# stevewongv/Sparse2Dense

Hardware: AMD Instinct MI355X
Metric: LiDAR frames/sec (fwd+bwd), 150k-pt 0.1m-voxel synthetic Waymo scene (higher is better)
Workload: dtype bf16 (sparse stack: bf16 storage; dense neck/head: bf16 NHWC activations; fp32 accumulate, statistics, master weights, optimizer)

## Files before the change

include/s2d.h:

```cpp
#ifndef S2D_H_
#define S2D_H_

#include <stddef.h>
#include <stdint.h>

#ifdef __cplusplus
extern "C" {
#endif

typedef void *s2d_stream_t;

#define S2D_OK 0
#define S2D_ERR_INVALID_ARG (-1)
#define S2D_ERR_UNSUPPORTED (-2)
#define S2D_ERR_CAPACITY (-3)
#define S2D_ERR_WORKSPACE (-4)
#define S2D_ERR_COMM (-5)

int s2d_version(void);
int s2d_last_error(char *buf, size_t buf_len);
int s2d_build_info(char *buf, size_t buf_len);

size_t s2d_voxelize_batch_workspace_bytes(int frames, const int64_t *point_offsets, int max_points, int max_voxels);
int s2d_voxelize_batch_run(const float *points, int frames, const int64_t *point_offsets, int ndim,
// ... 511 lines not shown
int s2d_comm_ranks(void);
int s2d_comm_shutdown(void);
int s2d_comm_allreduce_sum_f32(float *buf, int64_t count, s2d_stream_t stream);

int s2d_conv2d_pack_batch_bf16(int n, const float *const *weights, const int32_t *cin, const int32_t *cout, const int32_t *taps,
                               const int32_t *weight_nhwc, const int32_t *transpose_flip, void *const *packed_fwd, void *const *packed_dgrad,
                               s2d_stream_t stream);

int s2d_convt3d_mfma_fwd_stats_y16(const float *in, const void *packed, const float *bias, int batch, int cin, int cout, int d, int h, int w,
                                   void *out_bf16, float *stats_partial, s2d_stream_t stream);
int s2d_pointwise_conv_wgrad_norm_x16(const void *in_bf16, const float *in_scale_shift, const float *dout, int batch, int cin, int cout,
                                      int64_t positions, float *dweight, float *dbias, void *ws, size_t ws_bytes, s2d_stream_t stream);
int s2d_pcr_level_site_cache(void *buf, size_t bytes);
int s2d_pcr_level_fwd_y16_z16(const void *y, const float *bn_scale_shift, const float *head_params, const float *w2, const float *b2,
                              const int32_t *coors, const float *feats, int64_t m, int batch, int c, int co, int d, int h, int w, void *z_bf16,
                              float *z_stats, float *out8, void *ws, size_t ws_bytes, s2d_stream_t stream);
int s2d_pcr_level_bwd_sums_y16_z16(const void *y, const float *bn_scale_shift, const float *head_params, const int32_t *coors, const float *feats,
                                   int64_t m, int batch, int c, int d, int h, int w, const float *fwd_out8, const float *go_mask,
                                   const float *go_offset, const void *dz_bf16, const float *w2, int co, float *grads, float *bn_sums, void *ws,
                                   size_t ws_bytes, s2d_stream_t stream);
int s2d_pcr_level_bwd_apply_y16_d16_z16(const void *y, const float *bn_scale_shift, const float *head_params, const int32_t *coors,
                                        const float *feats, int64_t m, int batch, int c, int d, int h, int w, const float *fwd_out8,
                                        const float *go_mask, const float *go_offset, const void *dz_bf16, const float *w2, int co,
                                        const float *abd, void *dy_bf16, s2d_stream_t stream);
int s2d_pointwise_conv_wgrad_norm_x16_d16(const void *in_bf16, const float *in_scale_shift, const void *dout_bf16, int batch, int cin, int cout,
                                          int64_t positions, float *dweight, float *dbias, void *ws, size_t ws_bytes, s2d_stream_t stream);
int s2d_convt3d_mfma_x16_supported(int cin, int cout, int d, int h, int w);
int s2d_convt3d_mfma_fwd_stats_y16_norm_x16(const void *in_bf16, const float *in_scale_shift, const void *packed, const float *bias, int batch,
                                            int cin, int cout, int d, int h, int w, void *out_bf16, float *stats_partial, s2d_stream_t stream);
int s2d_convt3d_mfma_wgrad_d16_norm_x16(const void *in_bf16, const float *in_scale_shift, const void *dout_bf16, int batch, int cin, int cout,
                                        int d, int h, int w, float *dweight, void *ws, size_t ws_bytes, s2d_stream_t stream);
int s2d_convt3d_mfma_dgrad_d16_x16(const void *dout_bf16, const void *packed, int batch, int cin, int cout, int d, int h, int w, void *din_bf16,
                                   s2d_stream_t stream);
int s2d_bncm_bwd_reduce_x_typed(const void *dy, int dy_bf16, const void *x, int x_bf16, const float *scale, const float *shift, int batch, int c,
                                int64_t positions, float *sums, void *ws, size_t ws_bytes, s2d_stream_t stream);
int s2d_bncm_bwd_apply_x_typed(const void *dy, int dy_bf16, const void *x, int x_bf16, const float *scale, const float *shift, const float *a,
                               const float *b, const float *d, int batch, int c, int64_t positions, void *dx, int dx_bf16, s2d_stream_t stream);
int s2d_pcr_level_fwd_y16(const void *y, const float *bn_scale_shift, const float *head_params, const float *w2, const float *b2,
                          const int32_t *coors, const float *feats, int64_t m, int batch, int c, int co, int d, int h, int w, float *z,
                          float *z_stats, float *out8, void *ws, size_t ws_bytes, s2d_stream_t stream);
int s2d_pcr_level_bwd_sums_y16(const void *y, const float *bn_scale_shift, const float *head_params, const int32_t *coors, const float *feats,
                               int64_t m, int batch, int c, int d, int h, int w, const float *fwd_out8, const float *go_mask,
                               const float *go_offset, const float *dz, const float *w2, int co, float *grads, float *bn_sums, void *ws,
                               size_t ws_bytes, s2d_stream_t stream);
int s2d_pcr_level_bwd_apply_y16(const void *y, const float *bn_scale_shift, const float *head_params, const int32_t *coors, const float *feats,
                                int64_t m, int batch, int c, int d, int h, int w, const float *fwd_out8, const float *go_mask,
                                const float *go_offset, const float *dz, const float *w2, int co, const float *abd, float *dy,
                                s2d_stream_t stream);
int s2d_pcr_level_bwd_apply_y16_d16(const void *y, const float *bn_scale_shift, const float *head_params, const int32_t *coors, const float *feats,
                                    int64_t m, int batch, int c, int d, int h, int w, const float *fwd_out8, const float *go_mask,
                                    const float *go_offset, const float *dz, const float *w2, int co, const float *abd, void *dy_bf16,
                                    s2d_stream_t stream);

int s2d_pfn_supported(int ndim, int slots, int feats, int cout);
int s2d_pfn_blocks(int64_t pillars);
int s2d_pfn_bwd_cols(void);
int s2d_pfn_stats_f32(const float *voxels, const int32_t *num_points, const int32_t *coors, const float *weight, int64_t pillars,
                      int slots, int ndim, float vx, float vy, float x_offset, float y_offset, float *partial, s2d_stream_t stream);
int s2d_pfn_apply_max_f32(const float *voxels, const int32_t *num_points, const int32_t *coors, const float *weight, const float *scale,
                          const float *shift, int64_t pillars, int slots, int ndim, float vx, float vy, float x_offset, float y_offset,
                          float *out, uint8_t *argmax, s2d_stream_t stream);
int s2d_pfn_bwd_f32(const float *voxels, const int32_t *num_points, const int32_t *coors, const float *weight, const float *dout,
                    const uint8_t *argmax, int64_t pillars, int slots, int ndim, float vx, float vy, float x_offset, float y_offset,
                    float *partial, s2d_stream_t stream);

int s2d_pfn2_supported(int ndim, int slots, int feats, int c1, int c2);
// ... 177 lines not shown
```

sparse2dense_amd/_lib.py:

```python
import ctypes
import os

_HERE = os.path.dirname(os.path.abspath(__file__))
LIB_PATH = os.path.join(_HERE, "lib", "libs2d_hip.so")

c_i32p = ctypes.c_void_p
c_f32p = ctypes.c_void_p
_I3 = ctypes.c_int32 * 3
_PFN_GEO = [ctypes.c_int64, ctypes.c_int, ctypes.c_int, ctypes.c_float, ctypes.c_float, ctypes.c_float, ctypes.c_float]
_F3 = ctypes.c_float * 3
_F6 = ctypes.c_float * 6


class CenterTask(ctypes.Structure):
    _fields_ = [(n, ctypes.c_void_p) for n in ("hm_logit", "reg", "height", "dim", "vel", "rot", "hm", "ind", "mask", "cat", "anno_box", "p",
                                               "d_logit", "d_reg", "d_height", "d_dim", "d_vel", "d_rot")] + [("classes", ctypes.c_int)]

class CenterPredictTask(ctypes.Structure):
    _fields_ = [("map", ctypes.c_void_p * 6), ("channel_stride", ctypes.c_int64 * 6), ("pixel_stride", ctypes.c_int64 * 6),
                ("classes", ctypes.c_int), ("label_base", ctypes.c_int)]


class AnchorPredictTask(ctypes.Structure):
    _fields_ = [(n, ctypes.c_void_p) for n in ("box_preds", "cls_preds", "dir_cls_preds", "anchors")] + \
# ... 347 lines not shown
                                                 ctypes.c_int, ctypes.c_int, ctypes.c_int, ctypes.c_void_p, c_f32p, ctypes.c_void_p]),
    "s2d_conv2d3x3_wgrad_supported": (ctypes.c_int, [ctypes.c_int, ctypes.c_int]),
    "s2d_conv2d3x3_wgrad_workspace_bytes": (ctypes.c_size_t, [ctypes.c_int] * 6),
    "s2d_conv2d3x3_wgrad_nhwc_bf16": (ctypes.c_int, [ctypes.c_void_p, ctypes.c_void_p, ctypes.c_void_p] + [ctypes.c_int] * 6 +
                                      [c_f32p, c_f32p, ctypes.c_void_p, ctypes.c_size_t, ctypes.c_void_p]),
    "s2d_convt3d_k4s2p1_fwd_f32": (ctypes.c_int, [c_f32p, c_f32p, c_f32p, ctypes.c_int, ctypes.c_int, ctypes.c_int,
                                                  ctypes.c_int, ctypes.c_int, ctypes.c_int, c_f32p, ctypes.c_void_p]),
    "s2d_convt3d_k4s2p1_dgrad_f32": (ctypes.c_int, [c_f32p, c_f32p, ctypes.c_int, ctypes.c_int, ctypes.c_int,
                                                    ctypes.c_int, ctypes.c_int, ctypes.c_int, c_f32p, ctypes.c_void_p]),
    "s2d_convt3d_k4s2p1_wgrad_workspace_bytes": (ctypes.c_size_t, [ctypes.c_int] * 6),
    "s2d_convt3d_k4s2p1_wgrad_f32": (ctypes.c_int, [c_f32p, c_f32p, ctypes.c_int, ctypes.c_int, ctypes.c_int, ctypes.c_int,
                                                    ctypes.c_int, ctypes.c_int, c_f32p, ctypes.c_void_p, ctypes.c_size_t,
                                                    ctypes.c_void_p]),
    "s2d_bncm_workspace_bytes": (ctypes.c_size_t, [ctypes.c_int, ctypes.c_int, ctypes.c_int64]),
    "s2d_bncm_stats_f32": (ctypes.c_int, [c_f32p, ctypes.c_int, ctypes.c_int, ctypes.c_int64, c_f32p, ctypes.c_void_p,
                                          ctypes.c_size_t, ctypes.c_void_p]),
    "s2d_bncm_apply_f32": (ctypes.c_int, [c_f32p, c_f32p, c_f32p, ctypes.c_int, ctypes.c_int, ctypes.c_int,
                                          ctypes.c_int64, c_f32p, ctypes.c_void_p]),
    "s2d_bncm_bwd_reduce_f32": (ctypes.c_int, [c_f32p, c_f32p, c_f32p, ctypes.c_int, ctypes.c_int, ctypes.c_int,
                                               ctypes.c_int64, c_f32p, ctypes.c_void_p, ctypes.c_size_t, ctypes.c_void_p]),
    "s2d_bncm_bwd_reduce_x_f32": (ctypes.c_int, [c_f32p, c_f32p, c_f32p, c_f32p, ctypes.c_int, ctypes.c_int, ctypes.c_int64, c_f32p, ctypes.c_void_p,
                                                 ctypes.c_size_t, ctypes.c_void_p]),
    "s2d_bncm_bwd_apply_x_f32": (ctypes.c_int, [c_f32p] * 7 + [ctypes.c_int, ctypes.c_int, ctypes.c_int64, c_f32p, ctypes.c_void_p]),
    "s2d_bncm_bwd_reduce_x_typed": (ctypes.c_int, [ctypes.c_void_p, ctypes.c_int, ctypes.c_void_p, ctypes.c_int, c_f32p, c_f32p, ctypes.c_int, ctypes.c_int,
                                                   ctypes.c_int64, c_f32p, ctypes.c_void_p, ctypes.c_size_t, ctypes.c_void_p]),
    "s2d_bncm_bwd_apply_x_typed": (ctypes.c_int, [ctypes.c_void_p, ctypes.c_int, ctypes.c_void_p, ctypes.c_int, c_f32p, c_f32p, c_f32p, c_f32p, c_f32p,
                                                  ctypes.c_int, ctypes.c_int, ctypes.c_int64, ctypes.c_void_p, ctypes.c_int, ctypes.c_void_p]),
    "s2d_convt3d_mfma_x16_supported": (ctypes.c_int, [ctypes.c_int] * 5),
    "s2d_convt3d_mfma_dgrad_d16_x16": (ctypes.c_int, [ctypes.c_void_p, ctypes.c_void_p] + [ctypes.c_int] * 6 + [ctypes.c_void_p, ctypes.c_void_p]),
    "s2d_convt3d_mfma_fwd_stats_y16_norm_x16": (ctypes.c_int, [ctypes.c_void_p, c_f32p, ctypes.c_void_p, c_f32p] + [ctypes.c_int] * 6 +
                                                [ctypes.c_void_p, c_f32p, ctypes.c_void_p]),
    "s2d_convt3d_mfma_wgrad_d16_norm_x16": (ctypes.c_int, [ctypes.c_void_p, c_f32p, ctypes.c_void_p] + [ctypes.c_int] * 6 +
                                            [c_f32p, ctypes.c_void_p, ctypes.c_size_t, ctypes.c_void_p]),
    "s2d_pcr_level_site_cache": (ctypes.c_int, [ctypes.c_void_p, ctypes.c_size_t]),
    "s2d_pcr_level_fwd_y16_z16": (ctypes.c_int, [c_f32p, c_f32p, c_f32p, c_f32p, c_f32p, c_i32p, c_f32p, ctypes.c_int64] + [ctypes.c_int] * 6 +
                                  [ctypes.c_void_p, c_f32p, c_f32p, ctypes.c_void_p, ctypes.c_size_t, ctypes.c_void_p]),
    "s2d_pcr_level_bwd_sums_y16_z16": (ctypes.c_int, [c_f32p, c_f32p, c_f32p, c_i32p, c_f32p, ctypes.c_int64] + [ctypes.c_int] * 5 +
                                       [c_f32p, c_f32p, c_f32p, ctypes.c_void_p, c_f32p, ctypes.c_int, c_f32p, c_f32p, ctypes.c_void_p, ctypes.c_size_t,
                                        ctypes.c_void_p]),
    "s2d_pcr_level_bwd_apply_y16_d16_z16": (ctypes.c_int, [c_f32p, c_f32p, c_f32p, c_i32p, c_f32p, ctypes.c_int64] + [ctypes.c_int] * 5 +
                                            [c_f32p, c_f32p, c_f32p, ctypes.c_void_p, c_f32p, ctypes.c_int, c_f32p, ctypes.c_void_p, ctypes.c_void_p]),
    "s2d_pointwise_conv_wgrad_norm_x16_d16": (ctypes.c_int, [ctypes.c_void_p, c_f32p, ctypes.c_void_p, ctypes.c_int, ctypes.c_int, ctypes.c_int,
                                                              ctypes.c_int64, c_f32p, c_f32p, ctypes.c_void_p, ctypes.c_size_t, ctypes.c_void_p]),
    "s2d_space_depth2_nhwc_bf16": (ctypes.c_int, [ctypes.c_void_p] + [ctypes.c_int] * 5 + [ctypes.c_void_p, ctypes.c_void_p]),
    "s2d_bncm_bwd_apply_f32": (ctypes.c_int, [c_f32p, c_f32p, c_f32p, c_f32p, c_f32p, c_f32p, ctypes.c_int, ctypes.c_int,
                                              ctypes.c_int, ctypes.c_int64, c_f32p, ctypes.c_void_p]),
    "s2d_densify_bev_fwd_bf16": (ctypes.c_int, [ctypes.c_void_p, ctypes.c_int, c_i32p, ctypes.c_int64, ctypes.c_int, _I3,
                                                ctypes.c_int, ctypes.c_void_p, ctypes.c_void_p]),
    "s2d_densify_bev_bwd_bf16": (ctypes.c_int, [ctypes.c_void_p, c_i32p, ctypes.c_int64, ctypes.c_int, _I3, ctypes.c_int,
                                                ctypes.c_void_p, ctypes.c_int, ctypes.c_void_p]),
    "s2d_spconv_s16_wgrad": (ctypes.c_int, [ctypes.c_void_p, ctypes.c_int64, ctypes.c_void_p, c_i32p, ctypes.c_int64, ctypes.c_int,
                                            ctypes.c_int, ctypes.c_int, c_f32p, ctypes.c_void_p, ctypes.c_size_t, ctypes.c_void_p]),
    "s2d_densify_fwd_f32": (ctypes.c_int, [c_f32p, c_i32p, ctypes.c_int64, ctypes.c_int, _I3, ctypes.c_int, c_f32p,
                                           ctypes.c_void_p]),
    "s2d_densify_bwd_f32": (ctypes.c_int, [c_f32p, c_i32p, ctypes.c_int64, ctypes.c_int, _I3, ctypes.c_int, c_f32p,
                                           ctypes.c_void_p]),
    "s2d_anchor_assign_workspace_bytes": (ctypes.c_size_t, [ctypes.c_int, ctypes.c_int]),
    "s2d_anchor_assign": (ctypes.c_int, [c_f32p, c_i32p, ctypes.c_int, ctypes.c_int, c_f32p, ctypes.c_int64, ctypes.c_int, ctypes.c_int,
                                         ctypes.POINTER(ctypes.c_float), ctypes.POINTER(ctypes.c_float), c_i32p, c_f32p, c_f32p, ctypes.c_void_p,
                                         ctypes.c_size_t, ctypes.c_void_p]),
    "s2d_anchor_loss_workspace_bytes": (ctypes.c_size_t, [ctypes.c_int]),
    "s2d_anchor_loss_fwd": (ctypes.c_int, [c_f32p, c_f32p, c_f32p, c_i32p, c_f32p, c_f32p, ctypes.c_int, ctypes.c_int64, ctypes.c_int,
                                           ctypes.POINTER(ctypes.c_float), c_f32p, c_f32p, ctypes.c_void_p, ctypes.c_size_t, ctypes.c_void_p]),
    "s2d_anchor_loss_bwd": (ctypes.c_int, [c_f32p, c_f32p, c_f32p, c_i32p, c_f32p, c_f32p, ctypes.c_int, ctypes.c_int64, ctypes.c_int,
                                           ctypes.POINTER(ctypes.c_float), c_f32p, c_f32p, c_f32p, c_f32p, c_f32p, ctypes.c_void_p]),
    "s2d_anchor_decode": (ctypes.c_int, [c_f32p, c_f32p, c_f32p, c_f32p, ctypes.c_int, ctypes.c_int64, ctypes.c_int, ctypes.c_float, c_f32p,
# ... 158 lines not shown
```

sparse2dense_amd/csrc/convt3d_mfma.hip:

```cpp
#include "s2d_common.h"
#include <algorithm>
#include <cstdlib>

namespace s2d {

typedef float f32x4m __attribute__((ext_vector_type(4)));
typedef __bf16 bf16x8m __attribute__((ext_vector_type(8)));

constexpr unsigned CT_OOB = BUF_OOB;
__device__ __forceinline__ __amdgpu_buffer_rsrc_t ct_rsrc(const void *base, unsigned bytes) { return buf_rsrc(base, bytes); }
__device__ __forceinline__ f32x4m ct_load4(__amdgpu_buffer_rsrc_t r, unsigned voff, unsigned soff) { return buf_load4(r, voff, soff); }
typedef uint32_t u32x2m __attribute__((ext_vector_type(2)));
typedef uint32_t u32x3m __attribute__((ext_vector_type(3)));
typedef uint32_t u32x4m __attribute__((ext_vector_type(4)));
__device__ __forceinline__ u32x3m ct_load3u(__amdgpu_buffer_rsrc_t r, unsigned voff, unsigned soff) {
    return __builtin_bit_cast(u32x3m, __builtin_amdgcn_raw_buffer_load_b96(r, voff, soff, 0));
}
__device__ __forceinline__ u32x4m ct_load4u(__amdgpu_buffer_rsrc_t r, unsigned voff, unsigned soff) {
    return __builtin_bit_cast(u32x4m, __builtin_amdgcn_raw_buffer_load_b128(r, voff, soff, 0));
}
__device__ __forceinline__ u32x2m ct_load2u(__amdgpu_buffer_rsrc_t r, unsigned voff, unsigned soff) {
    return __builtin_bit_cast(u32x2m, __builtin_amdgcn_raw_buffer_load_b64(r, voff, soff, 0));
}
__device__ __forceinline__ uint32_t ct_hi_hi(uint32_t a, uint32_t b) { return __builtin_amdgcn_perm(b, a, 0x07060302u); }
// ... 1312 lines not shown
        const int a = f % CIT, g = f / CIT;
        const int ci = a * 16 + 4 * (ln >> 4) + reg, n_col = ln & 15;
        const int oc = n_col >> 2, okx = n_col & 3;
        if (ci < s.cin && oc < s.cout) dst[(((int64_t)ci * s.cout + oc) * 16 + g) * 4 + okx] = red[f4][ln];
    }
}

__global__ __launch_bounds__(256) void ct_slab_reduce_kernel(const float *__restrict__ partial, int n_slabs, int64_t size, float *__restrict__ out) {
    __shared__ float red[16][17];
    const int o = threadIdx.x & 15, sl = threadIdx.x >> 4;
    const int64_t i = (int64_t)blockIdx.x * 16 + o;
    float sum = 0.f;
    if (i < size)
        for (int sidx = sl; sidx < n_slabs; sidx += 16) sum += partial[(int64_t)sidx * size + i];
    red[sl][o] = sum;
    __syncthreads();
    if (sl == 0 && i < size) {
        float tot = 0.f;
#pragma unroll
        for (int k = 0; k < 16; ++k) tot += red[k][o];
        out[i] = tot;
    }
}

static bool ct_mfma_ok(int cin, int cout) { return (cin == 32 || cin == 16) && cout >= 1 && cout <= 32; }
static int ct_wgrad_blocks(int64_t rows) { return (int)(rows < 512 ? rows : 512); }
static bool ct_wgrad_is_narrow(int cout, int w) { return cout <= 4 && w % 8 == 0; }
static int ct_wgrad_blocks_for(int64_t rows, int cout, int w) {
    if (ct_wgrad_is_narrow(cout, w)) return (int)(rows < 1024 ? rows : 1024);
    if (w % 4 == 0) return (int)(rows < 128 ? rows : 128);
    return ct_wgrad_blocks(rows);
}

}

using namespace s2d;

extern "C" int s2d_convt3d_mfma_supported(int cin, int cout) { return ct_mfma_ok(cin, cout); }

extern "C" size_t s2d_convt3d_mfma_packed_elems(int cin, int cout) {
    if (!ct_mfma_ok(cin, cout)) return 0;
    const int nt_f = (cout + 15) / 16, nt_d = cin / 16, cop = cout <= 8 ? 8 : 32;
    return (size_t)8 * (cin == 32 ? 8 : 4) * nt_f * 512 + (size_t)2 * 16 * (cop == 32 ? 4 : 1) * nt_d * 512;
}

extern "C" int s2d_convt3d_mfma_pack_weights(const float *weight, int cin, int cout, void *packed, s2d_stream_t stream) {
    S2D_CHECK_ARG(weight && packed, "convt3d_mfma_pack: null argument");
    if (!ct_mfma_ok(cin, cout)) {
        set_error("convt3d_mfma: unsupported channels %d -> %d", cin, cout);
        return S2D_ERR_UNSUPPORTED;
    }
    const int nt_f = (cout + 15) / 16, nt_d = cin / 16, cop = cout <= 8 ? 8 : 32;
    const int n_f = 8 * (cin == 32 ? 8 : 4) * nt_f * 512, n_d = 16 * (cop == 32 ? 4 : 1) * nt_d * 512;
    hipStream_t st = (hipStream_t)stream;
    hipLaunchKernelGGL(ct_pack_fwd_kernel, dim3((n_f + 255) / 256), dim3(256), 0, st, weight, cin, cout, nt_f, (__bf16 *)packed);
    hipLaunchKernelGGL(ct_pack_dgrad_kernel, dim3((n_d + 255) / 256), dim3(256), 0, st, weight, cin, cout, cop, nt_d, 0, (__bf16 *)packed + n_f);
    hipLaunchKernelGGL(ct_pack_dgrad_kernel, dim3((n_d + 255) / 256), dim3(256), 0, st, weight, cin, cout, cop, nt_d, cout <= 4 ? 2 : 1,
                       (__bf16 *)packed + n_f + n_d);
    S2D_LAUNCH_CHECK();
    return S2D_OK;
}

static int ct_fwd_rows(int cin) { return cin == 32 ? 1 : 4; }

static bool ct_fwd_zslide(int cin) { return cin == 16; }

// ... 202 lines not shown
    if (!s2d_convt3d_mfma_d16_supported(cin, cout, d, h, w)) return S2D_ERR_UNSUPPORTED;
    const size_t need = s2d_convt3d_mfma_wgrad_workspace_bytes(batch, cin, cout, d, h, w);
    if (!ws || ws_bytes < need) {
        set_error("convt3d_mfma_wgrad_d16: workspace too small (%zu < %zu)", ws_bytes, need);
        return S2D_ERR_WORKSPACE;
    }
    return ct_wgrad_launch<__bf16>(in, (const __bf16 *)dout_bf16, batch, cin, cout, d, h, w, dweight, ws, (hipStream_t)stream);
}
extern "C" int s2d_convt3d_mfma_wgrad_d16_norm(const float *in, const float *in_scale_shift, const void *dout_bf16, int batch, int cin, int cout, int d,
                                               int h, int w, float *dweight, void *ws, size_t ws_bytes, s2d_stream_t stream) {
    S2D_CHECK_ARG(in && in_scale_shift && dout_bf16 && dweight && batch > 0, "convt3d_mfma_wgrad_d16_norm: bad argument");
    if (!s2d_convt3d_mfma_norm_supported(cin, cout, d, h, w)) return S2D_ERR_UNSUPPORTED;
    const size_t need = s2d_convt3d_mfma_wgrad_workspace_bytes(batch, cin, cout, d, h, w);
    if (!ws || ws_bytes < need) {
        set_error("convt3d_mfma_wgrad_d16_norm: workspace too small (%zu < %zu)", ws_bytes, need);
        return S2D_ERR_WORKSPACE;
    }
    return ct_wgrad_launch<__bf16>(in, (const __bf16 *)dout_bf16, batch, cin, cout, d, h, w, dweight, ws, (hipStream_t)stream, in_scale_shift);
}

extern "C" int s2d_convt3d_mfma_wgrad_d16_norm_x16(const void *in_bf16, const float *in_scale_shift, const void *dout_bf16, int batch, int cin, int cout,
                                                   int d, int h, int w, float *dweight, void *ws, size_t ws_bytes, s2d_stream_t stream) {
    S2D_CHECK_ARG(in_bf16 && in_scale_shift && dout_bf16 && dweight && batch > 0, "convt3d_mfma_wgrad_d16_norm_x16: bad argument");
    if (!s2d_convt3d_mfma_x16_supported(cin, cout, d, h, w)) return S2D_ERR_UNSUPPORTED;
    const size_t need = s2d_convt3d_mfma_wgrad_workspace_bytes(batch, cin, cout, d, h, w);
    if (!ws || ws_bytes < need) {
        set_error("convt3d_mfma_wgrad_d16_norm_x16: workspace too small (%zu < %zu)", ws_bytes, need);
        return S2D_ERR_WORKSPACE;
    }
    return ct_wgrad_launch<__bf16, __bf16>((const __bf16 *)in_bf16, (const __bf16 *)dout_bf16, batch, cin, cout, d, h, w, dweight, ws,
                                           (hipStream_t)stream, in_scale_shift);
}

namespace s2d {
constexpr int PW_CT = 4, PW_CIT = 32;

__global__ __launch_bounds__(256) void pw_wgrad_kernel(const float *__restrict__ x, const float *__restrict__ dy, int64_t p4, int batch, int cin,
                                                       int cout, int64_t quads_per_block, float *__restrict__ partial) {
    __shared__ float red[4][PW_CT * (PW_CIT + 1)];
    const int co0 = blockIdx.y * PW_CT, ci0 = blockIdx.z * PW_CIT;
    float acc[PW_CT][PW_CIT + 1];
#pragma unroll
    for (int c = 0; c < PW_CT; ++c)
#pragma unroll
        for (int i = 0; i <= PW_CIT; ++i) acc[c][i] = 0.f;
    const int64_t q0 = (int64_t)blockIdx.x * quads_per_block;
    const int64_t q1 = q0 + quads_per_block < p4 ? q0 + quads_per_block : p4;
    for (int n = 0; n < batch; ++n) {
        const float4 *xb = reinterpret_cast<const float4 *>(x) + (int64_t)n * cin * p4;
        const float4 *db = reinterpret_cast<const float4 *>(dy) + (int64_t)n * cout * p4;
        for (int64_t qd = q0 + threadIdx.x; qd < q1; qd += 256) {
            float4 g[PW_CT];
#pragma unroll
            for (int c = 0; c < PW_CT; ++c) {
                g[c] = co0 + c < cout ? db[(int64_t)(co0 + c) * p4 + qd] : float4{0.f, 0.f, 0.f, 0.f};
                acc[c][PW_CIT] += (g[c].x + g[c].y) + (g[c].z + g[c].w);
            }
#pragma unroll
            for (int i = 0; i < PW_CIT; ++i) {
                if (ci0 + i < cin) {
                    const float4 v = xb[(int64_t)(ci0 + i) * p4 + qd];
#pragma unroll
                    for (int c = 0; c < PW_CT; ++c)
                        acc[c][i] += (g[c].x * v.x + g[c].y * v.y) + (g[c].z * v.z + g[c].w * v.w);
                }
            }
// ... 268 lines not shown
```

sparse2dense_amd/dense3d.py:

```python
import ctypes

import os

import torch

from . import collective as _collective
import torch.nn.functional as F
from torch import nn

from . import _lib
from ._lib import check


def _ptr(t):
    return None if t is None else ctypes.c_void_p(t.data_ptr())


def _stream():
    return torch._C._cuda_getCurrentRawStream(torch.cuda.current_device())


def pointwise_conv(x, w2d, bias):
    lib = _lib.load()
    n, cin = x.shape[0], x.shape[1]
# ... 147 lines not shown
    import os
    if os.environ.get("S2D_PCR_PW_NHWC", "1") == "0":
        return False
    if not (isinstance(conv, PointwiseConv3d) and conv.bf16_compute and conv.kernel_size == (1, 1, 1) and conv.groups == 1):
        return False
    if not (torch.is_tensor(x) and x.is_cuda and x.dtype == torch.bfloat16 and x.dim() == 4 and x.is_contiguous(memory_format=torch.channels_last)):
        return False
    n, cd, h, w = x.shape
    co, c = conv.weight.shape[0], conv.weight.shape[1]
    cop = -(-co * depth // 64) * 64
    lib = _lib.load()
    return bool(cd == c * depth and (co * depth) % 8 == 0 and (h * w) % 4 == 0 and n <= 65535
                and lib.s2d_conv2d3x3_supported(cd, cop) and lib.s2d_conv2d3x3_supported(cop, cd))


def pw_conv_from_nhwc(x, conv, depth):
    return _PwConvNhwcFn.apply(x, conv.weight, conv.bias, depth)


def _convt_packed(weight):
    from .dense2d import cached_pack

    def build():
        lib = _lib.load()
        cin, cout = weight.shape[0], weight.shape[1]
        packed = torch.empty(lib.s2d_convt3d_mfma_packed_elems(cin, cout), dtype=torch.bfloat16, device=weight.device)
        wsrc = weight.detach().float().contiguous()
        launch = lambda: check(lib.s2d_convt3d_mfma_pack_weights(_ptr(wsrc), cin, cout, _ptr(packed), _stream()), "s2d_convt3d_mfma_pack_weights")
        launch()
        from .dense2d import register_repack
        register_repack(weight, [("convt3d_mfma",)], wsrc, launch)
        return packed
    return cached_pack(weight, ("convt3d_mfma",), build)


class _ConvT3dFn(torch.autograd.Function):
    @staticmethod
    def forward(ctx, x, weight, bias, bf16=False, bn_stats=False, out_bf16=False, in_norm=None):
        lib = _lib.load()
        x = x.contiguous()
        weight_param = weight
        weight = weight.contiguous()
        n, cin, d, h, w = x.shape
        cout = weight.shape[1]
        ctx.mfma = bool(bf16 and lib.s2d_convt3d_mfma_supported(cin, cout))
        ctx.in_norm = in_norm
        assert in_norm is None or (ctx.mfma and bn_stats and out_bf16 and lib.s2d_convt3d_mfma_norm_supported(cin, cout, d, h, w))
        x16 = x.dtype == torch.bfloat16
        assert not x16 or (in_norm is not None and lib.s2d_convt3d_mfma_x16_supported(cin, cout, d, h, w)), "bf16-stored input: the pre-norm x16 form only"
        out_bf16 = bool(out_bf16 and ctx.mfma and bn_stats)
        out = torch.empty((n, cout, 2 * d, 2 * h, 2 * w), dtype=torch.bfloat16 if out_bf16 else torch.float32, device=x.device)
        stats = None
        if ctx.mfma:
            partial = None
            if bn_stats:
                tiles = lib.s2d_convt3d_mfma_stats_tiles(n, cin, d, h, w)
                partial = torch.empty((tiles, 2, cout), dtype=torch.float32, device=x.device)
            if in_norm is not None:
                fwd_norm = lib.s2d_convt3d_mfma_fwd_stats_y16_norm_x16 if x16 else lib.s2d_convt3d_mfma_fwd_stats_y16_norm
                check(fwd_norm(_ptr(x), _ptr(in_norm), _ptr(_convt_packed(weight)), _ptr(bias), n, cin, cout, d, h, w,
                               _ptr(out), _ptr(partial), _stream()), "s2d_convt3d_mfma_fwd_stats_y16_norm")
            else:
                entry = lib.s2d_convt3d_mfma_fwd_stats_y16 if out_bf16 else lib.s2d_convt3d_mfma_fwd_stats
                check(entry(_ptr(x), _ptr(_convt_packed(weight)), _ptr(bias), n, cin, cout, d, h, w, _ptr(out), _ptr(partial), _stream()),
                      "s2d_convt3d_mfma_fwd_stats")
            if bn_stats:
                stats = torch.empty((2 * cout,), dtype=torch.float32, device=x.device)
                ws = _ws(lib.s2d_bn_partials_sum_workspace_bytes(partial.shape[0], cout), x.device)
                check(lib.s2d_bn_partials_sum_ws_f32(_ptr(partial), partial.shape[0], out.numel() // cout, cout, _ptr(stats), 0, _ptr(ws),
                                                     ws.numel(), _stream()), "s2d_bn_partials_sum_ws_f32")
        else:
            check(lib.s2d_convt3d_k4s2p1_fwd_f32(_ptr(x), _ptr(weight), _ptr(bias), n, cin, cout, d, h, w, _ptr(out), _stream()),
                  "s2d_convt3d_k4s2p1_fwd_f32")
        ctx.save_for_backward(x, weight)
        ctx.has_bias = bias is not None
        ctx.weight_p = weight_param
        if bn_stats:
            if stats is None:
                stats = _bncm_reduce("s2d_bncm_stats_f32", (_ptr(out),), n, cout, out[0, 0].numel(), x.device)
            ctx.mark_non_differentiable(stats)
            ctx.set_materialize_grads(False)
            return out, stats
        return out

    @staticmethod
    def backward(ctx, dout, *_unused, dout_sum=None):
        lib = _lib.load()
        x, weight = ctx.saved_tensors
        n, cin, d, h, w = x.shape
        cout = weight.shape[1]
        d16 = bool(dout.dtype == torch.bfloat16 and ctx.mfma and lib.s2d_convt3d_mfma_d16_supported(cin, cout, d, h, w))
        in_norm = getattr(ctx, "in_norm", None)
        assert in_norm is None or d16, "the input-norm fold runs with the bf16-stored gradient only"
        dout = dout.contiguous() if d16 else dout.float().contiguous()
        dx = dw = db = None
        x16 = x.dtype == torch.bfloat16
        assert not x16 or d16
        if ctx.needs_input_grad[0]:
            dx = torch.empty_like(x)
            if x16:
                check(lib.s2d_convt3d_mfma_dgrad_d16_x16(_ptr(dout), _ptr(_convt_packed(weight)), n, cin, cout, d, h, w, _ptr(dx), _stream()),
                      "s2d_convt3d_mfma_dgrad_d16_x16")
            elif d16:
                check(lib.s2d_convt3d_mfma_dgrad_d16(_ptr(dout), _ptr(_convt_packed(weight)), n, cin, cout, d, h, w, _ptr(dx), _stream()),
                      "s2d_convt3d_mfma_dgrad_d16")
            elif ctx.mfma:
                check(lib.s2d_convt3d_mfma_dgrad(_ptr(dout), _ptr(_convt_packed(weight)), n, cin, cout, d, h, w, _ptr(dx), _stream()),
                      "s2d_convt3d_mfma_dgrad")
            else:
                check(lib.s2d_convt3d_k4s2p1_dgrad_f32(_ptr(dout), _ptr(weight), n, cin, cout, d, h, w, _ptr(dx), _stream()),
                      "s2d_convt3d_k4s2p1_dgrad_f32")
        def wgrad():
            dw = torch.empty_like(weight)
            if _DEBUG_CT_WGRAD and in_norm is not None:
                from . import _debug
                return _debug.ct_wgrad_stand_in(_DEBUG_CT_WGRAD, dw, x.float() if x16 else x, dout, in_norm, (n, cin, cout, d, h, w),
                                                getattr(ctx, "_dbg_clones", None))
            if x16:
                ws = _ws(lib.s2d_convt3d_mfma_wgrad_workspace_bytes(n, cin, cout, d, h, w), x.device)
                check(lib.s2d_convt3d_mfma_wgrad_d16_norm_x16(_ptr(x), _ptr(in_norm), _ptr(dout), n, cin, cout, d, h, w, _ptr(dw), _ptr(ws), ws.numel(),
                                                              _stream()), "s2d_convt3d_mfma_wgrad_d16_norm_x16")
            elif d16 and in_norm is not None:
                ws = _ws(lib.s2d_convt3d_mfma_wgrad_workspace_bytes(n, cin, cout, d, h, w), x.device)
                check(lib.s2d_convt3d_mfma_wgrad_d16_norm(_ptr(x), _ptr(in_norm), _ptr(dout), n, cin, cout, d, h, w, _ptr(dw), _ptr(ws), ws.numel(),
                                                          _stream()), "s2d_convt3d_mfma_wgrad_d16_norm")
            elif d16:
                ws = _ws(lib.s2d_convt3d_mfma_wgrad_workspace_bytes(n, cin, cout, d, h, w), x.device)
                check(lib.s2d_convt3d_mfma_wgrad_d16(_ptr(x), _ptr(dout), n, cin, cout, d, h, w, _ptr(dw), _ptr(ws), ws.numel(), _stream()),
                      "s2d_convt3d_mfma_wgrad_d16")
            elif ctx.mfma:
                ws = _ws(lib.s2d_convt3d_mfma_wgrad_workspace_bytes(n, cin, cout, d, h, w), x.device)
                check(lib.s2d_convt3d_mfma_wgrad(_ptr(x), _ptr(dout), n, cin, cout, d, h, w, _ptr(dw), _ptr(ws), ws.numel(), _stream()),
                      "s2d_convt3d_mfma_wgrad")
            elif cin <= 32 and cout <= 32:
                ws = _ws(lib.s2d_convt3d_k4s2p1_wgrad_workspace_bytes(n, cin, cout, d, h, w), x.device)
                check(lib.s2d_convt3d_k4s2p1_wgrad_f32(_ptr(x), _ptr(dout), n, cin, cout, d, h, w, _ptr(dw), _ptr(ws),
                                                       ws.numel(), _stream()), "s2d_convt3d_k4s2p1_wgrad_f32")
            else:
                dp = F.pad(dout, (1, 1, 1, 1, 1, 1))
                xf = x.reshape(n, cin, -1)
                for kz in range(4):
                    for ky in range(4):
                        for kx in range(4):
                            sl = dp[:, :, kz:kz + 2 * d:2, ky:ky + 2 * h:2, kx:kx + 2 * w:2].reshape(n, cout, -1)
                            dw[:, :, kz, ky, kx] = torch.matmul(xf, sl.transpose(1, 2)).sum(0)
            return dw
        if ctx.needs_input_grad[1]:
            from . import side
            wp = getattr(ctx, "weight_p", None)
            if _DEBUG_CT_WGRAD == "clone_main" and in_norm is not None:
                ctx._dbg_clones = (x.clone(), dout.clone(), in_norm.clone())
            dw = side.run(wp, wgrad, x, dout, kind="pcr") if wp is not None else wgrad()
        if ctx.has_bias and ctx.needs_input_grad[2]:
            if dout_sum is not None:
                db = dout_sum
            elif d16:
                db = dout.float().sum(dim=(0, 2, 3, 4))
            elif dout[0, 0].numel() % 4 == 0:
                db = _bncm_reduce("s2d_bncm_stats_f32", (_ptr(dout),), n, cout, dout[0, 0].numel(), x.device)[:cout]
            else:
                db = dout.sum(dim=(0, 2, 3, 4))
        if not isinstance(ctx, torch.autograd.function.FunctionCtx):
            return dx, dw, db, None, None, None
        from . import side as _side
        return dx, _side.undefer(dw), db, None, None, None


def _hip_ok(x):
    return x.is_cuda and x.dtype == torch.float32 and not torch.is_autocast_enabled()


class PointwiseConv3d(nn.Conv3d):

    bf16_compute = False

    def forward(self, x):
        if _hip_ok(x) and self.kernel_size == (1, 1, 1) and self.stride == (1, 1, 1) and self.padding == (0, 0, 0) \
                and self.groups == 1:
            return _PwConvFn.apply(x, self.weight, self.bias, self.bf16_compute)
        return super().forward(x)
# ... 144 lines not shown
```

Before: 226.0.

## Fuse ConvTranspose3d dgrad and wgrad into one kernel for cin=16, cout=3

Adds a fused backward kernel for the stride-2 k4 transposed conv with 16 input and 3 output channels. It stages each dout row window into LDS once and uses it both for the data-gradient MFMA and for the weight-gradient MFMA, applying the input BN+ReLU on the fly. Per-tile weight partials go to scratch and are summed by a slab reduce. This removes a second read of dout and the separate wgrad launch, but it no longer runs wgrad on the side stream, which may lose overlap.

```diff
diff --git a/include/s2d.h b/include/s2d.h
--- a/include/s2d.h
+++ b/include/s2d.h
@@ -567,6 +567,11 @@
                                         int d, int h, int w, float *dweight, void *ws, size_t ws_bytes, s2d_stream_t stream);
 int s2d_convt3d_mfma_dgrad_d16_x16(const void *dout_bf16, const void *packed, int batch, int cin, int cout, int d, int h, int w, void *din_bf16,
                                    s2d_stream_t stream);
+int s2d_convt3d_mfma_bwd_fused_supported(int batch, int cin, int cout, int d, int h, int w);
+size_t s2d_convt3d_mfma_bwd_fused_scratch_bytes(int batch, int cin, int cout, int d, int h, int w);
+int s2d_convt3d_mfma_bwd_fused_d16_norm_x16(const void *in_bf16, const float *in_scale_shift, const void *dout_bf16, const void *packed, int batch,
+                                            int cin, int cout, int d, int h, int w, void *din_bf16, float *dweight, void *scratch,
+                                            size_t scratch_bytes, s2d_stream_t stream);
 int s2d_bncm_bwd_reduce_x_typed(const void *dy, int dy_bf16, const void *x, int x_bf16, const float *scale, const float *shift, int batch, int c,
                                 int64_t positions, float *sums, void *ws, size_t ws_bytes, s2d_stream_t stream);
 int s2d_bncm_bwd_apply_x_typed(const void *dy, int dy_bf16, const void *x, int x_bf16, const float *scale, const float *shift, const float *a,
diff --git a/sparse2dense_amd/_lib.py b/sparse2dense_amd/_lib.py
--- a/sparse2dense_amd/_lib.py
+++ b/sparse2dense_amd/_lib.py
@@ -403,6 +403,10 @@
                                                 [ctypes.c_void_p, c_f32p, ctypes.c_void_p]),
     "s2d_convt3d_mfma_wgrad_d16_norm_x16": (ctypes.c_int, [ctypes.c_void_p, c_f32p, ctypes.c_void_p] + [ctypes.c_int] * 6 +
                                             [c_f32p, ctypes.c_void_p, ctypes.c_size_t, ctypes.c_void_p]),
+    "s2d_convt3d_mfma_bwd_fused_supported": (ctypes.c_int, [ctypes.c_int] * 6),
+    "s2d_convt3d_mfma_bwd_fused_scratch_bytes": (ctypes.c_size_t, [ctypes.c_int] * 6),
+    "s2d_convt3d_mfma_bwd_fused_d16_norm_x16": (ctypes.c_int, [ctypes.c_void_p, c_f32p, ctypes.c_void_p, ctypes.c_void_p] + [ctypes.c_int] * 6 +
+                                                [ctypes.c_void_p, c_f32p, ctypes.c_void_p, ctypes.c_size_t, ctypes.c_void_p]),
     "s2d_pcr_level_site_cache": (ctypes.c_int, [ctypes.c_void_p, ctypes.c_size_t]),
     "s2d_pcr_level_fwd_y16_z16": (ctypes.c_int, [c_f32p, c_f32p, c_f32p, c_f32p, c_f32p, c_i32p, c_f32p, ctypes.c_int64] + [ctypes.c_int] * 6 +
                                   [ctypes.c_void_p, c_f32p, c_f32p, ctypes.c_void_p, ctypes.c_size_t, ctypes.c_void_p]),
diff --git a/sparse2dense_amd/csrc/convt3d_mfma.hip b/sparse2dense_amd/csrc/convt3d_mfma.hip
--- a/sparse2dense_amd/csrc/convt3d_mfma.hip
+++ b/sparse2dense_amd/csrc/convt3d_mfma.hip
@@ -1368,6 +1368,176 @@
     return ct_wgrad_blocks(rows);
 }
 
+constexpr int FB_TW = 128;
+constexpr int FB_RS = 136;
+constexpr int FB_PCS = 33;
+constexpr int FB_ROWS = 3 * 2 * 4 * 3;
+constexpr int FB_STAGE = 2 * 4 * 3 * FB_PCS;
+constexpr int FB_ITERS = (FB_STAGE + 255) / 256;
+
+__global__ __launch_bounds__(256) void ct_bwd_fused_n4_kernel(const __bf16 *__restrict__ x, const __bf16 *__restrict__ dout, const __bf16 *__restrict__ wp,
+                                                              const float *__restrict__ in_norm, CtDims s, int xtiles, int yc, int ychunks, int items,
+                                                              __bf16 *__restrict__ din, float *__restrict__ partial) {
+    __shared__ __attribute__((aligned(16))) uint32_t lds[FB_ROWS * FB_RS];
+    static_assert(FB_ROWS * FB_RS >= 64 * 64, "the accumulator fold reuses the ring");
+    const int t = threadIdx.x, lane = t & 63, wid = t >> 6;
+    const int r = lane & 15, q = lane >> 4;
+    const int item = xcd_tile(blockIdx.x, gridDim.x);
+    if (item >= items) return;
+    const int xt = item % xtiles;
+    int rem = item / xtiles;
+    const int hz = rem % s.d;
+    rem /= s.d;
+    const int chunk = rem % ychunks, n = rem / ychunks;
+    const int hy0 = chunk * yc, hy1 = min(s.h, hy0 + yc);
+    const int x0 = xt * FB_TW;
+    const int od = 2 * s.d, oh = 2 * s.h, ow = 2 * s.w;
+    const int64_t cells = (int64_t)s.d * s.h * s.w, oplane = (int64_t)od * oh * ow;
+    const unsigned xbytes = (unsigned)(s.cin * cells * 2), dbytes = (unsigned)(s.cout * oplane * 2);
+    const __amdgpu_buffer_rsrc_t xr = ct_rsrc(x + (int64_t)n * s.cin * cells, xbytes);
+    const __amdgpu_buffer_rsrc_t ir = ct_rsrc(din + (int64_t)n * s.cin * cells, xbytes);
+    const __amdgpu_buffer_rsrc_t dr = ct_rsrc(dout + (int64_t)n * s.cout * oplane, dbytes);
+    unsigned st_off[FB_ITERS], st_prev[FB_ITERS];
+    int st_lds[FB_ITERS], st_j[FB_ITERS];
+#pragma unroll
+    for (int it = 0; it < FB_ITERS; ++it) {
+        const int i = t + 256 * it;
+        const int p = i % FB_PCS, row = i / FB_PCS;
+        const int co = row % 3, zi = (row / 3) & 3, j = row / 12;
+        const int z = 2 * hz - 1 + zi, gw = x0 + 4 * p;
+        const bool rok = i < FB_STAGE && (unsigned)z < (unsigned)od && co < s.cout;
+        const unsigned base = (unsigned)(((int64_t)co * od + z) * oh * ow * 2) + (unsigned)gw * 4u;
+        st_off[it] = (rok && gw < s.w) ? base : CT_OOB;
+        st_prev[it] = (rok && gw > 0 && gw <= s.w) ? base - 4u : CT_OOB;
+        st_lds[it] = i < FB_STAGE ? row * FB_RS + 4 * p : -1;
+        st_j[it] = j;
+    }
+    u32x4m sv[FB_ITERS];
+    uint32_t sp[FB_ITERS];
+    auto stage_load = [&](int pair) {
+#pragma unroll
+        for (int it = 0; it < FB_ITERS; ++it) {
+            const int y = 2 * pair - 1 + st_j[it];
+            const bool yok = (unsigned)y < (unsigned)oh;
+            const unsigned yo = yok ? (unsigned)y * (unsigned)ow * 2u : 0u;
+            sv[it] = ct_load4u(dr, (yok && st_off[it] < CT_OOB) ? st_off[it] + yo : CT_OOB, 0);
+            sp[it] = __builtin_amdgcn_raw_buffer_load_b32(dr, (yok && st_prev[it] < CT_OOB) ? st_prev[it] + yo : CT_OOB, 0, 0);
+        }
+    };
+    auto stage_store = [&](int slot) {
+#pragma unroll
+        for (int it = 0; it < FB_ITERS; ++it) {
+            if (st_lds[it] < 0) continue;
+            const u32x4m o = {__builtin_amdgcn_alignbit(sv[it].x, sp[it], 16), __builtin_amdgcn_alignbit(sv[it].y, sv[it].x, 16),
+                              __builtin_amdgcn_alignbit(sv[it].z, sv[it].y, 16), __builtin_amdgcn_alignbit(sv[it].w, sv[it].z, 16)};
+            *reinterpret_cast<u32x4m *>(&lds[slot * (24 * FB_RS) + st_lds[it]]) = o;
+        }
+    };
+    bf16x8m wreg[8];
+#pragma unroll
+    for (int k8 = 0; k8 < 8; ++k8) wreg[k8] = *reinterpret_cast<const bf16x8m *>(wp + ((int64_t)k8 * 64 + lane) * 8);
+    const float nsc = in_norm[r], nsh = in_norm[s.cin + r];
+    const int cx = x0 + 32 * wid + 8 * q;
+    const unsigned xlane = cx < s.w ? (unsigned)(r * cells * 2) + (unsigned)cx * 2u : CT_OOB;
+    auto x_load = [&](int hy) { return ct_load4u(xr, xlane, (unsigned)(((int64_t)hz * s.h + hy) * s.w * 2)); };
+    f32x4m acc[16];
+#pragma unroll
+    for (int g = 0; g < 16; ++g) acc[g] = f32x4m{0.f, 0.f, 0.f, 0.f};
+    const int wco = min(r >> 2, 2), wkx = r & 3;
+    const uint32_t half_sel = (wkx & 1) ? 0x07060302u : 0x05040100u;
+    const bool wnext = wkx >= 2;
+    const int dco = 2 * (q & 1), dj = q >> 1;
+    const bool dhi = dco + 1 < s.cout;
+
+    stage_load(hy0);
+    stage_store(hy0 % 3);
+    stage_load(hy0 + 1);
+    stage_store((hy0 + 1) % 3);
+    u32x4m xc = x_load(hy0);
+    __syncthreads();
+#pragma unroll 1
+    for (int hy = hy0; hy < hy1; ++hy) {
+        const bool more = hy + 1 < hy1;
+        u32x4m xn = xc;
+        if (more) {
+            stage_load(hy + 2);
+            xn = x_load(hy + 1);
+        }
+        const int slot_lo = hy % 3, slot_hi = (hy + 1) % 3;
+        bf16x8m xa;
+        {
+            typedef short s16x2x __attribute__((ext_vector_type(2)));
+            const bool cv = cx < s.w;
+            const float sc = cv ? nsc : 0.f, sh = cv ? nsh : 0.f;
+            u32x4m o;
+#pragma unroll
+            for (int e = 0; e < 4; ++e) {
+                const float v0 = ct_fma_scalar(__uint_as_float(xc[e] << 16), sc, sh), v1 = ct_fma_scalar(__uint_as_float(xc[e] & 0xffff0000u), sc, sh);
+                const s16x2x r2 = __builtin_elementwise_max(__builtin_bit_cast(s16x2x, ct_cvt_pk_bf16(v0, v1)), s16x2x{0, 0});
+                o[e] = __builtin_bit_cast(uint32_t, r2);
+            }
+            xa = __builtin_bit_cast(bf16x8m, o);
+        }
+        f32x4m dacc[2] = {f32x4m{0.f, 0.f, 0.f, 0.f}, f32x4m{0.f, 0.f, 0.f, 0.f}};
+#pragma unroll
+        for (int k8 = 0; k8 < 8; ++k8) {
+            const int kz = k8 >> 1, slot = (k8 & 1) ? slot_hi : slot_lo;
+            const uint32_t *row = &lds[(((slot * 2 + dj) * 4 + kz) * 3 + dco) * FB_RS + 32 * wid + r];
+#pragma unroll
+            for (int mt = 0; mt < 2; ++mt) {
+                u32x4m pk;
+                pk.x = row[16 * mt];
+                pk.y = row[16 * mt + 1];
+                pk.z = dhi ? row[FB_RS + 16 * mt] : 0u;
+                pk.w = dhi ? row[FB_RS + 16 * mt + 1] : 0u;
+                dacc[mt] = __builtin_amdgcn_mfma_f32_16x16x32_bf16(__builtin_bit_cast(bf16x8m, pk), wreg[k8], dacc[mt], 0, 0, 0);
+            }
+        }
+#pragma unroll
+        for (int g = 0; g < 16; ++g) {
+            const int kz = g >> 2, ky = g & 3, slot = (ky >> 1) ? slot_hi : slot_lo;
+            const uint32_t *row = &lds[(((slot * 2 + (ky & 1)) * 4 + kz) * 3 + wco) * FB_RS + 32 * wid + 8 * q];
+            const u32x4m u0 = *reinterpret_cast<const u32x4m *>(row), u1 = *reinterpret_cast<const u32x4m *>(row + 4);
+            const uint32_t u8 = row[8];
+            const uint32_t w0 = wnext ? u0.y : u0.x, w1 = wnext ? u0.z : u0.y, w2 = wnext ? u0.w : u0.z, w3 = wnext ? u1.x : u0.w;
+            const uint32_t w4 = wnext ? u1.y : u1.x, w5 = wnext ? u1.z : u1.y, w6 = wnext ? u1.w : u1.z, w7 = wnext ? u8 : u1.w;
+            const u32x4m f = {__builtin_amdgcn_perm(w1, w0, half_sel), __builtin_amdgcn_perm(w3, w2, half_sel),
+                              __builtin_amdgcn_perm(w5, w4, half_sel), __builtin_amdgcn_perm(w7, w6, half_sel)};
+            acc[g] = __builtin_amdgcn_mfma_f32_16x16x32_bf16(xa, __builtin_bit_cast(bf16x8m, f), acc[g], 0, 0, 0);
+        }
+        const unsigned rowoff = (unsigned)(((int64_t)hz * s.h + hy) * s.w * 2);
+#pragma unroll
+        for (int mt = 0; mt < 2; ++mt) {
+            const int c0 = x0 + 32 * wid + 16 * mt + 4 * q;
+            const u32x2m o = {ct_cvt_pk_bf16(dacc[mt][0], dacc[mt][1]), ct_cvt_pk_bf16(dacc[mt][2], dacc[mt][3])};
+            buf_store2(ir, c0 < s.w ? (unsigned)(r * cells * 2) + (unsigned)c0 * 2u : CT_OOB, rowoff, __builtin_bit_cast(buf_f32x2, o));
+        }
+        if (more) stage_store((hy + 2) % 3);
+        xc = xn;
+        __syncthreads();
+    }
+    float *red = reinterpret_cast<float *>(lds);
+    for (int wv = 0; wv < 4; ++wv) {
+        if (wid == wv) {
+#pragma unroll
+            for (int g = 0; g < 16; ++g)
+#pragma unroll
+                for (int reg = 0; reg < 4; ++reg) {
+                    float *slot = &red[(g * 4 + reg) * 64 + lane];
+                    *slot = wv ? *slot + acc[g][reg] : acc[g][reg];
+                }
+        }
+        __syncthreads();
+    }
+    float *dst = partial + (int64_t)item * s.cin * s.cout * 64;
+    for (int e = t; e < 64 * 64; e += 256) {
+        const int ln = e % 64, f4 = e / 64, reg = f4 % 4, g = f4 / 4;
+        const int ci = 4 * (ln >> 4) + reg, n_col = ln & 15;
+        const int oc = n_col >> 2, okx = n_col & 3;
+        if (oc < s.cout) dst[(((int64_t)ci * s.cout + oc) * 16 + g) * 4 + okx] = red[f4 * 64 + ln];
+    }
+}
+
 }
 
 using namespace s2d;
@@ -1636,6 +1806,47 @@
                                            (hipStream_t)stream, in_scale_shift);
 }
 
+static int ct_fused_xtiles(int w) { return (w + FB_TW - 1) / FB_TW; }
+static int ct_fused_chunk_rows(int batch, int d, int h, int w) {
+    const int64_t strips = (int64_t)batch * d * ct_fused_xtiles(w);
+    const int want = (int)std::max<int64_t>(1, std::min<int64_t>(h, 1024 / strips));
+    return std::min(h, std::max((int)ceil_div(h, want), 4));
+}
+static int64_t ct_fused_items(int batch, int d, int h, int w) {
+    return (int64_t)batch * d * ct_fused_xtiles(w) * ceil_div(h, ct_fused_chunk_rows(batch, d, h, w));
+}
+extern "C" int s2d_convt3d_mfma_bwd_fused_supported(int batch, int cin, int cout, int d, int h, int w) {
+    return batch > 0 && cin == 16 && cout == 3 && s2d_convt3d_mfma_x16_supported(cin, cout, d, h, w) && (int64_t)cin * d * h * w * 2 < ((int64_t)1 << 31)
+           && ct_fused_items(batch, d, h, w) < (1 << 24);
+}
+extern "C" size_t s2d_convt3d_mfma_bwd_fused_scratch_bytes(int batch, int cin, int cout, int d, int h, int w) {
+    if (!s2d_convt3d_mfma_bwd_fused_supported(batch, cin, cout, d, h, w)) return 0;
+    return align_up((size_t)ct_fused_items(batch, d, h, w) * cin * cout * 64 * sizeof(float), 256);
+}
+extern "C" int s2d_convt3d_mfma_bwd_fused_d16_norm_x16(const void *in_bf16, const float *in_scale_shift, const void *dout_bf16, const void *packed,
+                                                       int batch, int cin, int cout, int d, int h, int w, void *din_bf16, float *dweight,
+                                                       void *scratch, size_t scratch_bytes, s2d_stream_t stream) {
+    S2D_CHECK_ARG(in_bf16 && in_scale_shift && dout_bf16 && packed && din_bf16 && dweight, "convt3d_mfma_bwd_fused: bad argument");
+    if (!s2d_convt3d_mfma_bwd_fused_supported(batch, cin, cout, d, h, w)) return S2D_ERR_UNSUPPORTED;
+    const size_t need = s2d_convt3d_mfma_bwd_fused_scratch_bytes(batch, cin, cout, d, h, w);
+    if (!scratch || scratch_bytes < need) {
+        set_error("convt3d_mfma_bwd_fused: scratch too small (%zu < %zu)", scratch_bytes, need);
+        return S2D_ERR_WORKSPACE;
+    }
+    CtDims s{batch, d, h, w, cin, cout};
+    hipStream_t st = (hipStream_t)stream;
+    const int xtiles = ct_fused_xtiles(w), yc = ct_fused_chunk_rows(batch, d, h, w), ychunks = (int)ceil_div(h, yc);
+    const int items = (int)ct_fused_items(batch, d, h, w);
+    const __bf16 *wd = (const __bf16 *)packed + (size_t)8 * 4 * 512 + (size_t)16 * 512;
+    float *partial = (float *)scratch;
+    hipLaunchKernelGGL(ct_bwd_fused_n4_kernel, dim3(xcd_grid(items)), dim3(256), 0, st, (const __bf16 *)in_bf16, (const __bf16 *)dout_bf16, wd,
+                       in_scale_shift, s, xtiles, yc, ychunks, items, (__bf16 *)din_bf16, partial);
+    const int64_t size = (int64_t)cin * cout * 64;
+    hipLaunchKernelGGL(ct_slab_reduce_kernel, dim3((unsigned)ceil_div(size, 16)), dim3(256), 0, st, partial, items, size, dweight);
+    S2D_LAUNCH_CHECK();
+    return S2D_OK;
+}
+
 namespace s2d {
 constexpr int PW_CT = 4, PW_CIT = 32;
 
diff --git a/sparse2dense_amd/dense3d.py b/sparse2dense_amd/dense3d.py
--- a/sparse2dense_amd/dense3d.py
+++ b/sparse2dense_amd/dense3d.py
@@ -203,6 +203,9 @@
         register_repack(weight, [("convt3d_mfma",)], wsrc, launch)
         return packed
     return cached_pack(weight, ("convt3d_mfma",), build)
+
+
+CT_FUSED_MIN_W = 128
 
 
 class _ConvT3dFn(torch.autograd.Function):
@@ -267,7 +270,16 @@
         dx = dw = db = None
         x16 = x.dtype == torch.bfloat16
         assert not x16 or d16
-        if ctx.needs_input_grad[0]:
+        fused = bool(x16 and in_norm is not None and ctx.needs_input_grad[0] and ctx.needs_input_grad[1] and not _DEBUG_CT_WGRAD
+                     and w >= CT_FUSED_MIN_W and lib.s2d_convt3d_mfma_bwd_fused_supported(n, cin, cout, d, h, w))
+        if fused:
+            dx = torch.empty_like(x)
+            dw = torch.empty_like(weight)
+            scratch = _ws(lib.s2d_convt3d_mfma_bwd_fused_scratch_bytes(n, cin, cout, d, h, w), x.device)
+            check(lib.s2d_convt3d_mfma_bwd_fused_d16_norm_x16(_ptr(x), _ptr(in_norm), _ptr(dout), _ptr(_convt_packed(weight)), n, cin, cout, d, h, w,
+                                                              _ptr(dx), _ptr(dw), _ptr(scratch), scratch.numel(), _stream()),
+                  "s2d_convt3d_mfma_bwd_fused_d16_norm_x16")
+        elif ctx.needs_input_grad[0]:
             dx = torch.empty_like(x)
             if x16:
                 check(lib.s2d_convt3d_mfma_dgrad_d16_x16(_ptr(dout), _ptr(_convt_packed(weight)), n, cin, cout, d, h, w, _ptr(dx), _stream()),
@@ -316,7 +328,7 @@
                             sl = dp[:, :, kz:kz + 2 * d:2, ky:ky + 2 * h:2, kx:kx + 2 * w:2].reshape(n, cout, -1)
                             dw[:, :, kz, ky, kx] = torch.matmul(xf, sl.transpose(1, 2)).sum(0)
             return dw
-        if ctx.needs_input_grad[1]:
+        if ctx.needs_input_grad[1] and not fused:
             from . import side
             wp = getattr(ctx, "weight_p", None)
             if _DEBUG_CT_WGRAD == "clone_main" and in_norm is not None:
```

After: 230.2, median of 4. 1.02x the previous value.
